# stdstu12/YUME

Measured on NVIDIA H100. Metric: latent_frames_per_sec, higher is better.
Workload: dtype bf16

## Files before the change

include/yume_b200.h:

```cpp
#ifndef YUME_B200_H_
#define YUME_B200_H_

#ifdef __cplusplus
extern "C" {
#endif

#define YB_OK 0
#define YB_ERR_ARG (-1)
#define YB_ERR_SHAPE (-2)
#define YB_ERR_ALIGNMENT (-3)
#define YB_ERR_NO_DRIVER (-4)
#define YB_ERR_TENSORMAP (-5)
#define YB_ERR_LAUNCH (-6)

int yb_abi_version(void);

#define YB_EPI_BF16 0
#define YB_EPI_GELU_BF16 1
#define YB_EPI_F32 2
#define YB_EPI_GATE_RES 3
#define YB_EPI_RES_BF16 5
#define YB_EPI_GELU_ERF_BF16 4

typedef struct yb_gemm_args {
// ... 15 lines not shown
  long long a_split_stride;
  const void* res;
  long long res_ld;
  int split_k;
  void* ws;
  long long ws_bytes;
} yb_gemm_args;
int yb_gemm_bf16(const yb_gemm_args* args, void* stream);
long long yb_gemm_workspace_bytes(int M, int N, int K, int epilogue, int cta_pair, int split_k);
int yb_gemm_splitk_plan(int tiles, int num_kb, int clusters, int split_k, int* out3);
int yb_gemm_plan(int M, int N, int sms, int* out4);

typedef struct yb_conv3d_args {
  unsigned int struct_bytes;
  int cta_pair;
  const void* xpad;
  const void* w;
  const void* bias;
  void* out;
  const void* res;
  long long ldo, res_ld;
  int T, H, W, Cp, Cout;
  int epilogue;
  int kt, kh, kw;
  int oob_zero_pad;
  int out_t_mul, out_t_add;
  int fuse_w;
  int stride_t, stride_hw;
} yb_conv3d_args;
int yb_conv3d_causal(const yb_conv3d_args* args, void* stream);
int yb_conv3d_plan(int T, int H, int W, int Cout, int kw, int fuse_w, int* out4);

int yb_ln_modulate(const void* x, long long ldx, void* out, long long ldo, int out_f32, const void* scale,
                   const void* shift, long long mod_ld, const void* tok_idx, const void* weight, const void* lnbias,
                   int L, int C, float eps, void* stream);

int yb_rmsnorm_rope(void* qk, long long ld, const void* weight, const void* rope, int rope_len, int L, int C, int D,
                    float eps, void* stream);
int yb_rmsnorm_rope_pieces(void* qk, long long ld, int piece_cols, long long piece_stride, const void* weight,
                           const void* rope, int rope_len, int L, int C, int D, float eps, void* stream);

int yb_qk_norm_rope(void* q, void* k, long long ld, int piece_cols, long long piece_stride, const void* wq, const void* wk,
                    const void* rope, int rope_len, int L, int C, int D, float eps, void* stream);

int yb_attention(const void* q, long long ldq, const void* k, long long ldk, const void* v, long long ldv, void* out,
                 long long ldo, int Lq, int Lk, int heads, float scale, int flags, void* stream);
int yb_attention_ex(const void* q, long long ldq, const void* k, long long ldk, const void* v, long long ldv, void* out,
                    long long ldo, int Lq, int Lk, int heads, float scale, int flags, void* ws, long long ws_bytes,
                    void* trace, void* stream);
#define YB_ATT_P_SMEM 1
#define YB_ATT_EMU_SHIFT 2
#define YB_ATT_ACCUMULATE 2
#define YB_ATT_SPLIT_SHIFT 4
int yb_attention_plan(int Lq, int Lk, int heads, int sms, int flags, int* out4);
long long yb_attention_workspace_bytes(int Lq, int Lk, int heads, int sms, int flags);
int yb_debug_force_split(int ns);
int yb_sp_scatter_qkv(const void* qkv, long long ld, const void* wq, const void* wk, const void* rope, int rope_len,
                      int L, int C, int D, float eps, void* const* peers, int world, int rank, int Lp, void* stream);
int yb_gemm_sp_qkv(const void* A, long long lda, const void* W, const void* bias, int Lp_rows, int C, int K, void* const* peers,
                   int world, int rank, int Lp, void* sums, void* stream);
int yb_sp_bcast_sums(void* local_sums, void* const* peer_tables, int world, int rank, int Lp, void* stream);
int yb_sp_post_norm_rope(void* buf, const void* sums, const void* wq, const void* wk, const void* rope, int rope_len, int L,
                         int Wh, int C, int D, float eps, void* stream);
int yb_attention_sp(const void* q, long long ldq, const void* k, long long ldk, const void* v, long long ldv,
                    void* const* out_peers, long long ldo, int Lq, int Lk, int heads, float scale, int world, int rank,
                    int Lp, int flags, void* ws, long long ws_bytes, void* stream);

int yb_patchify(const void* x, long long sc, long long sf, long long sh, long long sw, void* out, long long ldo,
                int Cin, int F, int H, int W, int ph, int pw, void* stream);

int yb_unpatchify(const void* y, long long ldy, void* out, int Cout, int F, int Hp, int Wp, int ph, int pw,
                  void* stream);

int yb_bcast_add(const void* a, const void* b, void* out, int R1, int R2, int n, void* stream);

int yb_sinusoidal(const void* t, void* out, int n, int dim, void* stream);

int yb_linear_f32_small(const void* in, const void* W, const void* bias, void* out, int M, int N, int K, int silu_in,
                        void* stream);

int yb_linear_f32(const void* in, long long ldi, const void* W, const void* bias, void* out, long long ldo, int M,
                  int N, int K, void* stream);

int yb_gn_stats(const void* x, long long ld, void* stats, long long N, int C, int G, void* stream);
int yb_vae_pad_act(const void* x, long long ldx, int Ts, int Hs, int Ws, int C, void* out, int Cp, int pad, int ft, int fh,
                   int fw, const void* stats, const void* gamma, const void* beta, int G, float eps, int silu,
                   void* stream);
int yb_masked_softmax(const void* S, long long ldS, void* P, long long ldP, int L, int hw, void* stream);
int yb_nchw_to_nhwc_bf16(const void* x, void* out, long long N, int Cn, int ldo, void* stream);
int yb_nhwc_to_nchw_f32(const void* x, long long ldx, void* out, long long N, int Cn, void* stream);
int yb_nhwc_to_nchw_f32_clamp(const void* x, long long ldx, void* out, long long N, int Cn, float lo, float hi, void* stream);
int yb_blend(const void* a, void* b, long long outer, int ea, int eb, int ext, long long inner, void* stream);

int yb_vae_assemble_tiles(const void* const* tile_ptrs, const int* th, const int* tw, const int* tlen, const int* tf0, int nt,
                          int ni, int nj, int C, int F, int H, int W, int row_limit, int blend_extent, int t_limit,
                          int t_blend_extent, void* out, void* stream);

int yb_vae_rms_act(const void* x, long long ldx, void* out, const void* gamma, int T, int Hs, int Ws, int C, int Cp, int up,
                   int silu, void* stream);
int yb_vae_dupup_add(void* main_, const void* x, int Ts, int Hs, int Ws, int in_c, int out_c, int ft, int fs, void* stream);
int yb_vae_unpatchify2_clamp(const void* y, long long ldy, void* out, int T, int H, int W, void* stream);
int yb_vae_avgdown_add(void* main_, const void* x, int T, int H, int W, int in_c, int out_c, int ft, int fs, void* stream);
int yb_vae_patchify2_bf16(const void* video, void* out, long long ldo, int T, int H, int W, void* stream);

int yb_umma_probe(const void* A, const void* B, void* D, int mode, void* stream);

// ... 5 lines not shown
```

yume_b200/_lib.py:

```python
from __future__ import annotations

import ctypes as C
from pathlib import Path

_LIB_PATH = Path(__file__).resolve().parent / "csrc" / "libyume_b200.so"

YB_EPI_BF16, YB_EPI_GELU_BF16, YB_EPI_F32, YB_EPI_GATE_RES, YB_EPI_GELU_ERF_BF16, YB_EPI_RES_BF16 = 0, 1, 2, 3, 4, 5
YB_ATT_P_SMEM, YB_ATT_ACCUMULATE = 1, 2
ABI_VERSION = 4
YB_ATT_EMU_SHIFT, YB_ATT_SPLIT_SHIFT = 2, 4

_ERRORS = {
    -1: "YB_ERR_ARG (null pointer / bad enum / non-positive size)",
    -2: "YB_ERR_SHAPE (shape not supported by the kernel)",
    -3: "YB_ERR_ALIGNMENT (pointer or stride not 16-byte aligned)",
    -4: "YB_ERR_NO_DRIVER (cuTensorMapEncodeTiled unavailable: no CUDA driver)",
    -5: "YB_ERR_TENSORMAP (driver rejected a TMA descriptor)",
    -6: "YB_ERR_LAUNCH (kernel launch failed)",
}


class YumeB200Error(RuntimeError):
    pass


class GemmArgs(C.Structure):

    _fields_ = [
        ("struct_bytes", C.c_uint), ("cta_pair", C.c_int),
        ("A", C.c_void_p), ("B", C.c_void_p), ("bias", C.c_void_p), ("out", C.c_void_p),
        ("gate", C.c_void_p), ("tok_idx", C.c_void_p),
        ("lda", C.c_longlong), ("ldb", C.c_longlong), ("ldo", C.c_longlong), ("gate_ld", C.c_longlong),
        ("M", C.c_int), ("N", C.c_int), ("K", C.c_int), ("epilogue", C.c_int), ("block_n", C.c_int),
        ("n_split", C.c_int), ("split_stride", C.c_longlong), ("a_split", C.c_int), ("a_split_stride", C.c_longlong),
        ("res", C.c_void_p), ("res_ld", C.c_longlong),
        ("split_k", C.c_int), ("ws", C.c_void_p), ("ws_bytes", C.c_longlong),
    ]


class Conv3dArgs(C.Structure):

    _fields_ = [
        ("struct_bytes", C.c_uint), ("cta_pair", C.c_int),
        ("xpad", C.c_void_p), ("w", C.c_void_p), ("bias", C.c_void_p), ("out", C.c_void_p), ("res", C.c_void_p),
        ("ldo", C.c_longlong), ("res_ld", C.c_longlong),
        ("T", C.c_int), ("H", C.c_int), ("W", C.c_int), ("Cp", C.c_int), ("Cout", C.c_int), ("epilogue", C.c_int),
        ("kt", C.c_int), ("kh", C.c_int), ("kw", C.c_int), ("oob_zero_pad", C.c_int), ("out_t_mul", C.c_int),
        ("out_t_add", C.c_int), ("fuse_w", C.c_int), ("stride_t", C.c_int), ("stride_hw", C.c_int),
    ]


_vp, _ll, _i, _f = C.c_void_p, C.c_longlong, C.c_int, C.c_float
SIGNATURES = {
    "yb_abi_version": (_i, []),
    "yb_gemm_bf16": (_i, [C.POINTER(GemmArgs), _vp]),
    "yb_conv3d_causal": (_i, [C.POINTER(Conv3dArgs), _vp]),
    "yb_gn_stats": (_i, [_vp, _ll, _vp, _ll, _i, _i, _vp]),
    "yb_vae_pad_act": (_i, [_vp, _ll, _i, _i, _i, _i, _vp, _i, _i, _i, _i, _i, _vp, _vp, _vp, _i, _f, _i, _vp]),
    "yb_masked_softmax": (_i, [_vp, _ll, _vp, _ll, _i, _i, _vp]),
    "yb_nchw_to_nhwc_bf16": (_i, [_vp, _vp, _ll, _i, _i, _vp]),
    "yb_nhwc_to_nchw_f32": (_i, [_vp, _ll, _vp, _ll, _i, _vp]),
# ... 71 lines not shown
```

yume_b200/csrc/attention.cu:

```cuda
#include "yb_host.h"
#include "yb_ptx.cuh"

namespace yb {

constexpr int ATT_THREADS = 384;
constexpr int ATT_TILE_BYTES = 128 * 128 * 2;

struct AttParams {
  __nv_bfloat16* out;
  long long ldo;
  int Lq, Lk;
  int nkv;
  int accumulate;
  __nv_bfloat16* out_peers[8];
  int sp_world, sp_rank, sp_Lp;
  float scale_log2;
  int nq, full_units, ns;
  float* ws_o;
  float* ws_ml;
};

template <bool P_SMEM>
struct AttCfg {
  static constexpr int NS = P_SMEM ? 4 : 5;
  static constexpr int Q_OFF = 0;
  static constexpr int P_OFF = ATT_TILE_BYTES;
  static constexpr int KV_OFF = P_SMEM ? 2 * ATT_TILE_BYTES : ATT_TILE_BYTES;
  static constexpr int BAR_OFF = KV_OFF + NS * ATT_TILE_BYTES;
  static constexpr int SMEM_BYTES = BAR_OFF + 256 + 1024;
  static_assert(SMEM_BYTES <= 227 * 1024, "shared memory budget");
};

template <bool P_SMEM>
__global__ void __launch_bounds__(ATT_THREADS, 1)
attention_kernel(const __grid_constant__ CUtensorMap tmQ, const __grid_constant__ CUtensorMap tmK,
                 const __grid_constant__ CUtensorMap tmV, const AttParams p) {
  using Cfg = AttCfg<P_SMEM>;
  constexpr int NS = Cfg::NS;
  extern __shared__ uint8_t smem_raw[];
  uint8_t* smem = reinterpret_cast<uint8_t*>((reinterpret_cast<uintptr_t>(smem_raw) + 1023) & ~uintptr_t(1023));
  uint64_t* q_full = reinterpret_cast<uint64_t*>(smem + Cfg::BAR_OFF);
  uint64_t* q_empty = q_full + 1;
  uint64_t* kv_full = q_empty + 1;
  uint64_t* kv_empty = kv_full + NS;

  const int warp = threadIdx.x >> 5;
  const int lane = threadIdx.x & 31;
  int unit = blockIdx.x, kv_begin = 0, nkv = p.nkv;
  if (static_cast<int>(blockIdx.x) >= p.full_units) {
    const int r = blockIdx.x - p.full_units;
    unit = p.full_units + r / p.ns;
    const int per = (((p.nkv + p.ns - 1) / p.ns) + 1) & ~1;
    kv_begin = (r % p.ns) * per;
    nkv = min(per, p.nkv - kv_begin);
  }
  const int head = unit / p.nq;
  const int q0 = (unit - head * p.nq) * 256;
  const int nx = q0 + 128 < p.Lq ? 2 : 1;

  if (threadIdx.x == 0) {
    tma_prefetch_desc(&tmQ);
    tma_prefetch_desc(&tmK);
    tma_prefetch_desc(&tmV);
    mbar_init(q_full, 1);
    mbar_init(q_empty, 8);
    for (int i = 0; i < NS; ++i) {
      mbar_init(&kv_full[i], 1);
      mbar_init(&kv_empty[i], 8);
    }
    fence_barrier_init();
  }
  __syncthreads();

  if (warp < 4) {
    setmaxnreg_dec<40>();
    if (warp == 0 && lane == 0) {
      int it = 0;
      for (int X = 0; X < nx; ++X) {
        if (X == 1) mbar_wait(q_empty, 0);
        mbar_arrive_expect_tx(q_full, ATT_TILE_BYTES);
        for (int s = 0; s < 2; ++s)
          tma_load_2d(smem + Cfg::Q_OFF + s * 16384, &tmQ, q_full, head * 128 + s * 64, q0 + X * 128);
        for (int jj = 0; jj < 2 * nkv; ++jj, ++it) {
          const int slot = it % NS;
          mbar_wait(&kv_empty[slot], ((it / NS) & 1) ^ 1);
          mbar_arrive_expect_tx(&kv_full[slot], ATT_TILE_BYTES);
          const CUtensorMap* tm = (jj & 1) ? &tmV : &tmK;
          uint8_t* dst = smem + Cfg::KV_OFF + slot * ATT_TILE_BYTES;
          const int j = kv_begin + (jj >> 1);
          tma_load_2d(dst, tm, &kv_full[slot], head * 128, j * 128);
          tma_load_2d(dst + 16384, tm, &kv_full[slot], head * 128 + 64, j * 128);
        }
      }
    }
  } else {
    setmaxnreg_inc<232>();
    const int wg = (warp >> 2) - 1;
    const int q4 = lane >> 2, c2 = 2 * (lane & 3);
    const int row_a = wg * 64 + (warp & 3) * 16 + q4;
    const float sc = p.scale_log2;
    const uint32_t sQ = smem_u32(smem + Cfg::Q_OFF) + wg * 64 * 128;
    const uint32_t sP = smem_u32(smem + Cfg::P_OFF) + wg * 16384;
    int it = 0;
    for (int X = 0; X < nx; ++X) {
      mbar_wait(q_full, X);
      float o[64];
#pragma unroll
      for (int i = 0; i < 64; ++i) o[i] = 0.f;
      float m0 = -INFINITY, m1 = -INFINITY, l0 = 0.f, l1 = 0.f;
      for (int j = 0; j < nkv; ++j, it += 2) {
        const int slot_k = it % NS, slot_v = (it + 1) % NS;
        mbar_wait(&kv_full[slot_k], (it / NS) & 1);
        const uint32_t sK = smem_u32(smem + Cfg::KV_OFF + slot_k * ATT_TILE_BYTES);
        float s[64];
#pragma unroll
        for (int i = 0; i < 64; ++i) s[i] = 0.f;
        wgmma_fence();
#pragma unroll
        for (int kk = 0; kk < 8; ++kk) {
          const uint32_t off = (kk >> 2) * 16384 + (kk & 3) * 32;
          wgmma_ss_acc64<0>(s, make_smem_desc_sw128(sQ + off, 16, 1024), make_smem_desc_sw128(sK + off, 16, 1024), kk != 0);
        }
        wgmma_commit();
        wgmma_wait<0>();
        fence_regs(s);
        __syncwarp();
        if (lane == 0) {
          mbar_arrive(&kv_empty[slot_k]);
          if (j == nkv - 1) mbar_arrive(q_empty);
        }
        const int kv_rem = p.Lk - (kv_begin + j) * 128;
        if (kv_rem < 128) {
#pragma unroll
          for (int i = 0; i < 64; ++i)
            if (8 * (i >> 2) + c2 + (i & 1) >= kv_rem) s[i] = -INFINITY;
        }
        float mx0 = -INFINITY, mx1 = -INFINITY;
#pragma unroll
        for (int g = 0; g < 16; ++g) {
          mx0 = fmaxf(mx0, fmaxf(s[4 * g], s[4 * g + 1]));
          mx1 = fmaxf(mx1, fmaxf(s[4 * g + 2], s[4 * g + 3]));
        }
        mx0 = fmaxf(mx0, __shfl_xor_sync(0xffffffffu, mx0, 1));
        mx0 = fmaxf(mx0, __shfl_xor_sync(0xffffffffu, mx0, 2));
        mx1 = fmaxf(mx1, __shfl_xor_sync(0xffffffffu, mx1, 1));
        mx1 = fmaxf(mx1, __shfl_xor_sync(0xffffffffu, mx1, 2));
        const float mn0 = fmaxf(m0, mx0 * sc), mn1 = fmaxf(m1, mx1 * sc);
        const float al0 = fast_exp2(m0 - mn0), al1 = fast_exp2(m1 - mn1);
        m0 = mn0;
        m1 = mn1;
        l0 *= al0;
        l1 *= al1;
#pragma unroll
        for (int g = 0; g < 16; ++g) {
          o[4 * g] *= al0;
          o[4 * g + 1] *= al0;
          o[4 * g + 2] *= al1;
          o[4 * g + 3] *= al1;
        }
        uint32_t pa[8][4];
#pragma unroll
        for (int kk = 0; kk < 8; ++kk) {
          float e[8];
#pragma unroll
          for (int i = 0; i < 8; ++i) e[i] = fast_exp2(s[8 * kk + i] * sc - ((i & 2) ? m1 : m0));
          l0 += (e[0] + e[1]) + (e[4] + e[5]);
          l1 += (e[2] + e[3]) + (e[6] + e[7]);
          pa[kk][0] = pack_bf16x2(e[0], e[1]);
          pa[kk][1] = pack_bf16x2(e[2], e[3]);
          pa[kk][2] = pack_bf16x2(e[4], e[5]);
          pa[kk][3] = pack_bf16x2(e[6], e[7]);
        }
        if (P_SMEM) {
          const int ra = row_a - wg * 64, rb = ra + 8;
#pragma unroll
          for (int kk = 0; kk < 8; ++kk) {
            uint8_t* slab = smem + Cfg::P_OFF + wg * 16384 + (kk >> 2) * 8192;
            const int k0 = (kk & 3) * 16 + c2, k1 = k0 + 8;
            *reinterpret_cast<uint32_t*>(slab + ra * 128 + (((k0 >> 3) ^ (ra & 7)) << 4) + (k0 & 7) * 2) = pa[kk][0];
            *reinterpret_cast<uint32_t*>(slab + rb * 128 + (((k0 >> 3) ^ (rb & 7)) << 4) + (k0 & 7) * 2) = pa[kk][1];
            *reinterpret_cast<uint32_t*>(slab + ra * 128 + (((k1 >> 3) ^ (ra & 7)) << 4) + (k1 & 7) * 2) = pa[kk][2];
            *reinterpret_cast<uint32_t*>(slab + rb * 128 + (((k1 >> 3) ^ (rb & 7)) << 4) + (k1 & 7) * 2) = pa[kk][3];
          }
          fence_proxy_async_smem();
          named_bar_sync(1 + wg, 128);
        }
        mbar_wait(&kv_full[slot_v], ((it + 1) / NS) & 1);
        const uint32_t sV = smem_u32(smem + Cfg::KV_OFF + slot_v * ATT_TILE_BYTES);
        wgmma_fence();
#pragma unroll
        for (int kk = 0; kk < 8; ++kk) {
          const uint64_t vdesc = make_smem_desc_sw128(sV + kk * 2048, 16384, 1024);
          if (P_SMEM)
            wgmma_ss_acc64<1>(o, make_smem_desc_sw128(sP + (kk >> 2) * 8192 + (kk & 3) * 32, 16, 1024), vdesc, 1u);
          else
            wgmma_rs_n128_tb(o, pa[kk], vdesc, 1u);
        }
        wgmma_commit();
        wgmma_wait<0>();
        fence_regs(o);
        __syncwarp();
        if (lane == 0) mbar_arrive(&kv_empty[slot_v]);
      }
      l0 += __shfl_xor_sync(0xffffffffu, l0, 1);
      l0 += __shfl_xor_sync(0xffffffffu, l0, 2);
      l1 += __shfl_xor_sync(0xffffffffu, l1, 1);
      l1 += __shfl_xor_sync(0xffffffffu, l1, 2);

#pragma unroll
      for (int h = 0; h < 2; ++h) {
        const int row_t = X * 128 + row_a + 8 * h;
        const float m = h ? m1 : m0, l = h ? l1 : l0;
        if (static_cast<int>(blockIdx.x) >= p.full_units) {
          const long long prow = static_cast<long long>(blockIdx.x - p.full_units) * 256 + row_t;
          float* wo = p.ws_o + prow * 128;
#pragma unroll
          for (int g = 0; g < 16; ++g) *reinterpret_cast<float2*>(wo + 8 * g + c2) = make_float2(o[4 * g + 2 * h], o[4 * g + 2 * h + 1]);
          if ((lane & 3) == 0) *reinterpret_cast<float2*>(p.ws_ml + prow * 2) = make_float2(m, l);
          continue;
        }
        const int q_row = q0 + row_t;
        if (q_row >= p.Lq) continue;
        __nv_bfloat16* orow = p.out + static_cast<long long>(q_row) * p.ldo + head * 128;
        if (p.sp_world > 1) {
          const int owner = q_row / p.sp_Lp;
          const int t = q_row - owner * p.sp_Lp;
          if (owner < p.sp_world)
            orow = p.out_peers[owner] + (static_cast<long long>(p.sp_rank) * p.sp_Lp + t) * p.ldo + head * 128;
        }
        const float inv = 1.0f / l;
#pragma unroll
        for (int g = 0; g < 16; ++g) {
          uint32_t* dst = reinterpret_cast<uint32_t*>(orow + 8 * g + c2);
          float v0 = o[4 * g + 2 * h] * inv, v1 = o[4 * g + 2 * h + 1] * inv;
          if (p.accumulate) {
            const float2 prev = __bfloat1622float2(*reinterpret_cast<const __nv_bfloat162*>(dst));
            v0 += prev.x;
            v1 += prev.y;
          }
          *dst = pack_bf16x2(v0, v1);
        }
      }
    }
  }
}

__global__ void __launch_bounds__(256) attention_combine_kernel(const AttParams p, int tail_units) {
  const int gw = blockIdx.x * 8 + (threadIdx.x >> 5);
  const int lane = threadIdx.x & 31;
  if (gw >= tail_units * 256) return;
  const int tu = gw >> 8, r = gw & 255;
  const int unit = p.full_units + tu;
  const int head = unit / p.nq;
  const int q_row = (unit - head * p.nq) * 256 + r;
  if (q_row >= p.Lq) return;
  float M = -INFINITY;
  for (int sgm = 0; sgm < p.ns; ++sgm) M = fmaxf(M, p.ws_ml[((static_cast<long long>(tu) * p.ns + sgm) * 256 + r) * 2]);
  float4 acc = make_float4(0.f, 0.f, 0.f, 0.f);
  float lsum = 0.f;
  for (int sgm = 0; sgm < p.ns; ++sgm) {
    const long long prow = (static_cast<long long>(tu) * p.ns + sgm) * 256 + r;
    const float2 ml = *reinterpret_cast<const float2*>(p.ws_ml + prow * 2);
    const float w = exp2f(ml.x - M);
    const float4 o = *reinterpret_cast<const float4*>(p.ws_o + prow * 128 + lane * 4);
    acc.x += o.x * w; acc.y += o.y * w; acc.z += o.z * w; acc.w += o.w * w;
    lsum += ml.y * w;
  }
  const float inv = 1.0f / lsum;
  __nv_bfloat16* orow = p.out + static_cast<long long>(q_row) * p.ldo + head * 128;
  if (p.sp_world > 1) {
    const int owner = q_row / p.sp_Lp;
    const int t = q_row - owner * p.sp_Lp;
    if (owner < p.sp_world)
      orow = p.out_peers[owner] + (static_cast<long long>(p.sp_rank) * p.sp_Lp + t) * p.ldo + head * 128;
  }
  *reinterpret_cast<uint2*>(orow + lane * 4) = make_uint2(pack_bf16x2(acc.x * inv, acc.y * inv), pack_bf16x2(acc.z * inv, acc.w * inv));
}

static void attention_plan(int units, int nkv, int sms, bool allowed, int force_ns, int* full_units, int* tail, int* ns) {
  *full_units = units;
  *tail = 0;
  *ns = 1;
  if (!allowed || force_ns == 1) return;
  if (force_ns >= 2 && nkv >= 2 * force_ns) {
    *tail = units;
    *ns = force_ns;
  } else if (force_ns == 0 && units > sms && units % sms != 0 && 2 * (units % sms) <= sms && nkv >= 16) {
    *tail = units % sms;
    *ns = sms / *tail < 4 ? sms / *tail : 4;
  }
  while (*ns > 1 && (*ns - 1) * ((((nkv + *ns - 1) / *ns) + 1) & ~1) >= nkv) --*ns;
  if (*ns == 1) *tail = 0;
  *full_units = units - *tail;
}

static size_t split_workspace_bytes(size_t ctas) { return ctas * 256 * 130 * sizeof(float); }

static int g_debug_force_split = 0;

template <bool P_SMEM>
static int launch_attention(const CUtensorMap& tmQ, const CUtensorMap& tmK, const CUtensorMap& tmV,
                            AttParams p, int heads, cudaStream_t stream, int force_ns, void* ws, long long ws_bytes) {
  using Cfg = AttCfg<P_SMEM>;
  auto kern = attention_kernel<P_SMEM>;
  static bool attr_set[kMaxDevices] = {false};
  if (int rc = ensure_dynamic_smem(kern, Cfg::SMEM_BYTES, attr_set, "attention")) return rc;
  if (force_ns == 0 && g_debug_force_split >= 1 && g_debug_force_split <= 4) force_ns = g_debug_force_split;
  p.nq = (p.Lq + 255) / 256;
  const int units = p.nq * heads;
  int tail = 0;
  p.ws_o = p.ws_ml = nullptr;
  const bool allowed = !p.accumulate && ws != nullptr;
  attention_plan(units, p.nkv, sm_count(), allowed, force_ns, &p.full_units, &tail, &p.ns);
  if (tail > 0) {
    const size_t ctas = static_cast<size_t>(tail) * p.ns;
    if (ws_bytes < 0 || static_cast<size_t>(ws_bytes) < split_workspace_bytes(ctas) || (reinterpret_cast<uintptr_t>(ws) & 0xF)) {
      p.full_units = units;
      tail = 0;
      p.ns = 1;
    } else {
      p.ws_o = static_cast<float*>(ws);
      p.ws_ml = p.ws_o + ctas * 256 * 128;
    }
  }
  kern<<<p.full_units + tail * p.ns, ATT_THREADS, Cfg::SMEM_BYTES, stream>>>(tmQ, tmK, tmV, p);
  int rc = check_launch("attention");
  if (rc || tail == 0) return rc;
  attention_combine_kernel<<<tail * 32, 256, 0, stream>>>(p, tail);
  return check_launch("attention_combine");
}

static int dispatch_attention(const void* q, long long ldq, const void* k, long long ldk, const void* v, long long ldv,
                              AttParams p, int heads, cudaStream_t stream, int flags, void* ws, long long ws_bytes) {
  const int force_ns = (flags >> YB_ATT_SPLIT_SHIFT) & 7;
  if (force_ns > 4) return YB_ERR_ARG;
  if ((flags >> YB_ATT_EMU_SHIFT) & 3) return YB_ERR_ARG;
  CUtensorMap tmQ, tmK, tmV;
  const uint64_t cols = static_cast<uint64_t>(heads) * 128;
  int rc = make_tmap_bf16_2d(&tmQ, q, p.Lq, cols, ldq, 128, 64);
  if (rc) return rc;
  rc = make_tmap_bf16_2d(&tmK, k, p.Lk, cols, ldk, 128, 64);
  if (rc) return rc;
  rc = make_tmap_bf16_2d(&tmV, v, p.Lk, cols, ldv, 128, 64);
  if (rc) return rc;
  if (flags & YB_ATT_P_SMEM) return launch_attention<true>(tmQ, tmK, tmV, p, heads, stream, force_ns, ws, ws_bytes);
  return launch_attention<false>(tmQ, tmK, tmV, p, heads, stream, force_ns, ws, ws_bytes);
}

}

extern "C" int yb_debug_force_split(int ns) {
  if (ns < 0 || ns > 4) return YB_ERR_ARG;
  yb::g_debug_force_split = ns;
  return YB_OK;
}

extern "C" int yb_attention_plan(int Lq, int Lk, int heads, int sms, int flags, int* out4) {
  if (Lq <= 0 || Lk <= 0 || heads <= 0 || sms <= 0 || !out4) return YB_ERR_ARG;
  int force_ns = (flags >> YB_ATT_SPLIT_SHIFT) & 7;
  if (force_ns > 4) return YB_ERR_ARG;
  if (force_ns == 0 && yb::g_debug_force_split >= 1) force_ns = yb::g_debug_force_split;
  const int nkv = (Lk + 127) / 128;
  int full_units, tail, ns;
  yb::attention_plan(((Lq + 255) / 256) * heads, nkv, sms, !(flags & YB_ATT_ACCUMULATE), force_ns, &full_units, &tail, &ns);
  out4[0] = full_units;
  out4[1] = tail;
  out4[2] = ns;
  out4[3] = ns > 1 ? ((((nkv + ns - 1) / ns) + 1) & ~1) : nkv;
  return YB_OK;
}

extern "C" long long yb_attention_workspace_bytes(int Lq, int Lk, int heads, int sms, int flags) {
  int plan[4];
  if (yb_attention_plan(Lq, Lk, heads, sms, flags, plan)) return -1;
  return static_cast<long long>(yb::split_workspace_bytes(static_cast<size_t>(plan[1]) * plan[2]));
}

extern "C" int yb_attention_ex(const void* q, long long ldq, const void* k, long long ldk, const void* v,
                               long long ldv, void* out, long long ldo, int Lq, int Lk, int heads, float scale,
                               int flags, void* ws, long long ws_bytes, void* trace, void* stream_) {
  using namespace yb;
  if (!q || !k || !v || !out) return YB_ERR_ARG;
  if (Lq <= 0 || Lk <= 0 || heads <= 0) return YB_ERR_ARG;
  if ((ldo % 8) != 0 || (reinterpret_cast<uintptr_t>(out) & 0xF)) return YB_ERR_ALIGNMENT;
  AttParams p;
  p.out = static_cast<__nv_bfloat16*>(out);
  p.ldo = ldo;
  p.Lq = Lq;
  p.Lk = Lk;
  p.nkv = (Lk + 127) / 128;
  p.accumulate = (flags & YB_ATT_ACCUMULATE) ? 1 : 0;
  (void)trace;
  p.sp_world = 1;
  p.sp_rank = 0;
  p.sp_Lp = 0;
  p.scale_log2 = scale * 1.4426950408889634f;
  return dispatch_attention(q, ldq, k, ldk, v, ldv, p, heads, reinterpret_cast<cudaStream_t>(stream_), flags, ws, ws_bytes);
}

// ... 28 lines not shown
```

yume_b200/ops.py:

```python
from __future__ import annotations

import ctypes as C
import math
from typing import Optional

import torch

from . import _lib
from ._lib import (YB_ATT_ACCUMULATE, YB_ATT_P_SMEM, YB_EPI_BF16, YB_EPI_F32, YB_EPI_GATE_RES, YB_EPI_GELU_BF16,
                   YB_EPI_GELU_ERF_BF16, YB_EPI_RES_BF16, Conv3dArgs, GemmArgs, YumeB200Error, check)

__all__ = [
    "gemm", "ln_modulate", "rmsnorm_rope", "qk_norm_rope", "flop_count", "attention", "patchify", "unpatchify", "sinusoidal",
    "resize_bicubic_normalize",
    "linear_f32_small", "linear_f32", "umma_probe", "launch_count", "reset_launch_count",
    "YB_EPI_BF16", "YB_EPI_GELU_BF16", "YB_EPI_F32", "YB_EPI_GATE_RES", "YB_EPI_GELU_ERF_BF16", "bcast_add",
    "YB_ATT_P_SMEM", "YB_ATT_ACCUMULATE",
]

_launches = 0
_flops = 0.0


def flop_count() -> float:
    return _flops


def launch_count() -> int:
    return _launches


def reset_launch_count() -> None:
    global _launches, _flops
    _launches = 0
    _flops = 0.0


def _stream() -> int:
    return torch.cuda.current_stream().cuda_stream


def _ptr(t: Optional[torch.Tensor]) -> Optional[int]:
    return None if t is None else t.data_ptr()


def _need(t: torch.Tensor, dtype, name: str) -> None:
    if not t.is_cuda:
        raise YumeB200Error(f"{name} must be a CUDA tensor (yume_b200 has no CPU path)")
    if t.dtype != dtype:
        raise YumeB200Error(f"{name} must be {dtype}, got {t.dtype}")
    if t.stride(-1) != 1:
        raise YumeB200Error(f"{name} must be contiguous in its last dimension")


def gemm(a: torch.Tensor, w: torch.Tensor, bias: Optional[torch.Tensor], out: torch.Tensor, epilogue: int,
         gate: Optional[torch.Tensor] = None, tok_idx: Optional[torch.Tensor] = None, block_n: int = 0,
         n_split: int = 0, split_stride: int = 0, a_split: int = 0, a_split_stride: int = 0,
         shape: Optional[tuple] = None, res: Optional[torch.Tensor] = None, cta_pair: int = 0, split_k: Optional[int] = None) -> torch.Tensor:
    global _launches, _flops
    _need(a, torch.bfloat16, "a")
    _need(w, torch.bfloat16, "w")
    N, K2 = w.shape
    if shape is not None:
        M, K = shape
    else:
        M, K = a.shape
    if K2 != K:
        raise YumeB200Error(f"gemm K mismatch: {K} vs {K2}")
    want = torch.bfloat16 if epilogue in (YB_EPI_BF16, YB_EPI_GELU_BF16, YB_EPI_GELU_ERF_BF16, YB_EPI_RES_BF16) else torch.float32
    if res is not None:
# ... 67 lines not shown
    check(_lib.load().yb_rmsnorm_rope_pieces(qk.data_ptr(), qk.stride(0), piece_cols, piece_stride, weight.data_ptr(),
                                             _ptr(rope), rope_len or 0, L, Cdim, head_dim, eps, _stream()),
          "yb_rmsnorm_rope")
    _launches += 1
    return qk


def qk_norm_rope(q: torch.Tensor, k: torch.Tensor, wq: torch.Tensor, wk: torch.Tensor, rope: Optional[torch.Tensor],
                 head_dim: int, eps: float = 1e-6, rope_len: Optional[int] = None, pieces: Optional[tuple] = None) -> None:
    global _launches
    _need(q, torch.bfloat16, "q")
    _need(k, torch.bfloat16, "k")
    _need(wq, torch.float32, "wq")
    _need(wk, torch.float32, "wk")
    if q.stride(0) != k.stride(0):
        raise YumeB200Error("q and k must share their row stride")
    if pieces is not None:
        L, Cdim, piece_cols, piece_stride = pieces
    else:
        if q.shape != k.shape:
            raise YumeB200Error("q and k must have the same shape")
        L, Cdim = q.shape
        piece_cols, piece_stride = Cdim, 0
    if rope is not None:
        _need(rope, torch.float32, "rope")
        if not rope.is_contiguous() or rope.shape[-1] != 2 or rope.shape[-2] != head_dim // 2:
            raise YumeB200Error("rope must be contiguous f32 [L, D/2, 2]")
        if rope_len is None:
            rope_len = rope.shape[0]
    check(_lib.load().yb_qk_norm_rope(q.data_ptr(), k.data_ptr(), q.stride(0), piece_cols, piece_stride, wq.data_ptr(),
                                      wk.data_ptr(), _ptr(rope), rope_len or 0, L, Cdim, head_dim, eps, _stream()),
          "yb_qk_norm_rope")
    _launches += 1


_sm_counts = {}


def _sms(device: torch.device) -> int:
    idx = device.index if device.index is not None else torch.cuda.current_device()
    n = _sm_counts.get(idx)
    if n is None:
        n = _sm_counts[idx] = torch.cuda.get_device_properties(idx).multi_processor_count
    return n


def _attention_ws(Lq: int, Lk: int, heads: int, flags: int, device: torch.device):
    nbytes = _lib.load().yb_attention_workspace_bytes(Lq, Lk, heads, _sms(device), flags)
    if nbytes <= 0:
        return None, 0
    return torch.empty(nbytes, dtype=torch.uint8, device=device), nbytes


def attention(q: torch.Tensor, k: torch.Tensor, v: torch.Tensor, out: torch.Tensor, heads: int,
              scale: Optional[float] = None, variant: int = 0, accumulate: bool = False,
              split: int = 0) -> torch.Tensor:
    global _launches, _flops
    for n, t in (("q", q), ("k", k), ("v", v), ("out", out)):
        _need(t, torch.bfloat16, n)
    Lq, Lk = q.shape[0], k.shape[0]
    if q.shape[1] != heads * 128 or k.shape[1] != heads * 128 or v.shape[1] != heads * 128:
        raise YumeB200Error("attention supports head_dim 128 only")
    if scale is None:
        scale = 1.0 / math.sqrt(128.0)
    flags = (YB_ATT_P_SMEM if variant == 1 else 0) | (YB_ATT_ACCUMULATE if accumulate else 0) | ((split & 7) << 4)
    if variant not in (0, 1):
        raise YumeB200Error("attention variant must be 0 or 1")
    ws, ws_bytes = _attention_ws(Lq, Lk, heads, flags, q.device)
    check(_lib.load().yb_attention_ex(q.data_ptr(), q.stride(0), k.data_ptr(), k.stride(0), v.data_ptr(), v.stride(0),
                                      out.data_ptr(), out.stride(0), Lq, Lk, heads, scale, flags, _ptr(ws), ws_bytes, None,
                                      _stream()), "yb_attention")
    _launches += 1
    _flops += 4.0 * Lq * Lk * heads * 128
    return out


def patchify(x: torch.Tensor, out: torch.Tensor, ph: int, pw: int) -> torch.Tensor:
    global _launches
    if not x.is_cuda or x.dtype != torch.float32:
        raise YumeB200Error("patchify input must be a CUDA float32 tensor")
    _need(out, torch.bfloat16, "out")
    Cin, F, H, W = x.shape
    sc, sf, sh, sw = x.stride()
    check(_lib.load().yb_patchify(x.data_ptr(), sc, sf, sh, sw, out.data_ptr(), out.stride(0), Cin, F, H, W, ph, pw,
                                  _stream()), "yb_patchify")
    _launches += 1
    return out


def resize_bicubic_normalize(x: torch.Tensor, out: torch.Tensor, mean: torch.Tensor, std: torch.Tensor) -> torch.Tensor:
    global _launches
    if not x.is_cuda or x.dtype != torch.float32 or x.dim() != 3:
        raise YumeB200Error("resize_bicubic_normalize input must be a CUDA float32 [C, H, W] tensor")
    _need(out, torch.float32, "out")
    Cn, H, W = x.shape
    S = out.shape[-1]
    if not out.is_contiguous() or tuple(out.shape) != (Cn, S, S):
        raise YumeB200Error(f"resize_bicubic_normalize out must be a contiguous [{Cn}, S, S], got {tuple(out.shape)}")
    for name, t in (("mean", mean), ("std", std)):
        _need(t, torch.float32, name)
        if t.numel() != Cn or not t.is_contiguous():
            raise YumeB200Error(f"resize_bicubic_normalize {name} must be a contiguous f32 [{Cn}]")
    sc, sh, sw = x.stride()
    check(_lib.load().yb_resize_bicubic_normalize(x.data_ptr(), sc, sh, sw, Cn, H, W, out.data_ptr(), S, mean.data_ptr(),
                                                  std.data_ptr(), _stream()), "yb_resize_bicubic_normalize")
    _launches += 1
    return out


def unpatchify(y: torch.Tensor, out: torch.Tensor, F: int, Hp: int, Wp: int, ph: int, pw: int) -> torch.Tensor:
    global _launches
    _need(y, torch.float32, "y")
    _need(out, torch.float32, "out")
    Cout = out.shape[0]
    check(_lib.load().yb_unpatchify(y.data_ptr(), y.stride(0), out.data_ptr(), Cout, F, Hp, Wp, ph, pw, _stream()),
          "yb_unpatchify")
    _launches += 1
    return out


# ... 207 lines not shown


def _ptr_array(ptrs):
    arr = (C.c_void_p * len(ptrs))(*[int(p) for p in ptrs])
    return arr


def sp_scatter_qkv(qkv: torch.Tensor, wq: torch.Tensor, wk: torch.Tensor, rope: Optional[torch.Tensor], rope_len: int,
                   head_dim: int, eps: float, peer_ptrs, rank: int, Lp: int) -> None:
    global _launches
    _need(qkv, torch.bfloat16, "qkv")
    L, C3 = qkv.shape
    check(_lib.load().yb_sp_scatter_qkv(qkv.data_ptr(), qkv.stride(0), wq.data_ptr(), wk.data_ptr(), _ptr(rope), rope_len,
                                        L, C3 // 3, head_dim, eps, _ptr_array(peer_ptrs), len(peer_ptrs), rank, Lp,
                                        _stream()), "yb_sp_scatter_qkv")
    _launches += 1


def gemm_sp_qkv(h: torch.Tensor, w_qkv: torch.Tensor, b_qkv: torch.Tensor, peer_ptrs, rank: int, Lp: int,
                sums: torch.Tensor) -> None:
    global _launches, _flops
    _need(h, torch.bfloat16, "h")
    _need(w_qkv, torch.bfloat16, "w_qkv")
    _need(b_qkv, torch.float32, "b_qkv")
    _need(sums, torch.float32, "sums")
    if not w_qkv.is_contiguous():
        raise YumeB200Error("gemm_sp_qkv weight must be contiguous")
    M, K = h.shape
    C3 = w_qkv.shape[0]
    check(_lib.load().yb_gemm_sp_qkv(h.data_ptr(), h.stride(0), w_qkv.data_ptr(), b_qkv.data_ptr(), M, C3 // 3, K,
                                     _ptr_array(peer_ptrs), len(peer_ptrs), rank, Lp, sums.data_ptr(), _stream()),
          "yb_gemm_sp_qkv")
    _launches += 1
    _flops += 2.0 * M * C3 * K


def sp_bcast_sums(local: torch.Tensor, peer_table_ptrs, rank: int, Lp: int) -> None:
    global _launches
    check(_lib.load().yb_sp_bcast_sums(local.data_ptr(), _ptr_array(peer_table_ptrs), len(peer_table_ptrs), rank, Lp, _stream()),
          "yb_sp_bcast_sums")
    _launches += 1


def sp_post_norm_rope(buf: torch.Tensor, sums: torch.Tensor, wq: torch.Tensor, wk: torch.Tensor, rope: Optional[torch.Tensor],
                      rope_len: int, L: int, Wh: int, Cdim: int, head_dim: int, eps: float) -> None:
    global _launches
    _need(buf, torch.bfloat16, "buf")
    check(_lib.load().yb_sp_post_norm_rope(buf.data_ptr(), sums.data_ptr(), wq.data_ptr(), wk.data_ptr(), _ptr(rope), rope_len, L,
                                           Wh, Cdim, head_dim, eps, _stream()), "yb_sp_post_norm_rope")
    _launches += 1


def attention_sp(q: torch.Tensor, k: torch.Tensor, v: torch.Tensor, out_peer_ptrs, ldo: int, heads: int, rank: int,
                 Lp: int, scale: Optional[float] = None) -> None:
    global _launches, _flops
    for n, t in (("q", q), ("k", k), ("v", v)):
        _need(t, torch.bfloat16, n)
    if scale is None:
        scale = 1.0 / math.sqrt(128.0)
    flags = 0
    ws, ws_bytes = _attention_ws(q.shape[0], k.shape[0], heads, flags, q.device)
    check(_lib.load().yb_attention_sp(q.data_ptr(), q.stride(0), k.data_ptr(), k.stride(0), v.data_ptr(), v.stride(0),
                                      _ptr_array(out_peer_ptrs), ldo, q.shape[0], k.shape[0], heads, scale,
                                      len(out_peer_ptrs), rank, Lp, flags, _ptr(ws), ws_bytes, _stream()), "yb_attention_sp")
    _launches += 1
    _flops += 4.0 * q.shape[0] * k.shape[0] * heads * 128


def vae_rms_act(x: torch.Tensor, dims, out: torch.Tensor, gamma: Optional[torch.Tensor], up: int = 1, silu: bool = True) -> torch.Tensor:
    global _launches
    _need(x, torch.bfloat16, "x")
    _need(out, torch.bfloat16, "out")
    T, Hs, Ws = dims
    if not out.is_contiguous():
        raise YumeB200Error("vae_rms_act output must be contiguous")
    check(_lib.load().yb_vae_rms_act(x.data_ptr(), x.stride(0), out.data_ptr(), _ptr(gamma), T, Hs, Ws, x.shape[1],
                                     out.shape[-1], up, 1 if silu else 0, _stream()), "yb_vae_rms_act")
    _launches += 1
    return out


def vae_dupup_add(main: torch.Tensor, x: torch.Tensor, dims, in_c: int, out_c: int, ft: int, fs: int) -> torch.Tensor:
    global _launches
    _need(main, torch.bfloat16, "main")
    _need(x, torch.bfloat16, "x")
    if not (main.is_contiguous() and x.is_contiguous()):
        raise YumeB200Error("vae_dupup_add needs dense tensors")
    check(_lib.load().yb_vae_dupup_add(main.data_ptr(), x.data_ptr(), dims[0], dims[1], dims[2], in_c, out_c, ft, fs,
                                       _stream()), "yb_vae_dupup_add")
    _launches += 1
    return main


def vae_avgdown_add(main: torch.Tensor, x: torch.Tensor, dims, in_c: int, out_c: int, ft: int, fs: int) -> torch.Tensor:
    global _launches
    _need(main, torch.bfloat16, "main")
    _need(x, torch.bfloat16, "x")
    if not (main.is_contiguous() and x.is_contiguous()) or x.shape[-1] != in_c or main.shape[-1] != out_c:
        raise YumeB200Error("vae_avgdown_add needs dense [.., in_c] / [.., out_c] tensors")
    check(_lib.load().yb_vae_avgdown_add(main.data_ptr(), x.data_ptr(), dims[0], dims[1], dims[2], in_c, out_c, ft, fs,
                                         _stream()), "yb_vae_avgdown_add")
    _launches += 1
    return main


def vae_patchify2_bf16(video: torch.Tensor, out: torch.Tensor) -> torch.Tensor:
    global _launches
    _need(video, torch.float32, "video")
    _need(out, torch.bfloat16, "out")
    if video.dim() != 4 or video.shape[0] != 3 or not video.is_contiguous() or not out.is_contiguous():
        raise YumeB200Error("vae_patchify2_bf16: video must be a contiguous [3, T, H, W]")
    _, T, H, W = video.shape
    check(_lib.load().yb_vae_patchify2_bf16(video.data_ptr(), out.data_ptr(), out.shape[-1], T, H, W, _stream()),
# ... 14 lines not shown
```

Before: 39.05.

## Pipeline attention QK^T of next tile with PV of previous tile

Adds a software-pipelined attention schedule in which the QK^T wgmma for tile j is issued together with the PV wgmma for tile j-1, so softmax overlaps with tensor-core work. P is passed through shared memory in this path. The old serial schedule stays available behind a new SERIAL flag, and the default variant now runs the pipelined P-in-smem kernel instead of the register-P kernel. This adds shared-memory stores of P and extra synchronization, and may raise register pressure.

```diff
diff --git a/include/yume_b200.h b/include/yume_b200.h
--- a/include/yume_b200.h
+++ b/include/yume_b200.h
@@ -91,6 +91,7 @@
 #define YB_ATT_EMU_SHIFT 2
 #define YB_ATT_ACCUMULATE 2
 #define YB_ATT_SPLIT_SHIFT 4
+#define YB_ATT_SERIAL 128
 int yb_attention_plan(int Lq, int Lk, int heads, int sms, int flags, int* out4);
 long long yb_attention_workspace_bytes(int Lq, int Lk, int heads, int sms, int flags);
 int yb_debug_force_split(int ns);
diff --git a/yume_b200/_lib.py b/yume_b200/_lib.py
--- a/yume_b200/_lib.py
+++ b/yume_b200/_lib.py
@@ -6,7 +6,7 @@
 _LIB_PATH = Path(__file__).resolve().parent / "csrc" / "libyume_b200.so"
 
 YB_EPI_BF16, YB_EPI_GELU_BF16, YB_EPI_F32, YB_EPI_GATE_RES, YB_EPI_GELU_ERF_BF16, YB_EPI_RES_BF16 = 0, 1, 2, 3, 4, 5
-YB_ATT_P_SMEM, YB_ATT_ACCUMULATE = 1, 2
+YB_ATT_P_SMEM, YB_ATT_ACCUMULATE, YB_ATT_SERIAL = 1, 2, 128
 ABI_VERSION = 4
 YB_ATT_EMU_SHIFT, YB_ATT_SPLIT_SHIFT = 2, 4
 
diff --git a/yume_b200/csrc/attention.cu b/yume_b200/csrc/attention.cu
--- a/yume_b200/csrc/attention.cu
+++ b/yume_b200/csrc/attention.cu
@@ -31,10 +31,100 @@
   static_assert(SMEM_BYTES <= 227 * 1024, "shared memory budget");
 };
 
+__device__ __forceinline__ void att_issue_qk(float (&s)[64], uint32_t sQ, uint32_t sK) {
+#pragma unroll
+  for (int i = 0; i < 64; ++i) s[i] = 0.f;
+  wgmma_fence();
+#pragma unroll
+  for (int kk = 0; kk < 8; ++kk) {
+    const uint32_t off = (kk >> 2) * 16384 + (kk & 3) * 32;
+    wgmma_ss_acc64<0>(s, make_smem_desc_sw128(sQ + off, 16, 1024), make_smem_desc_sw128(sK + off, 16, 1024), kk != 0);
+  }
+  wgmma_commit();
+}
+
+__device__ __forceinline__ void att_softmax(float (&s)[64], int kv_rem, int c2, float sc, float& m0, float& m1, float& l0,
+                                            float& l1, float& al0, float& al1, uint32_t (&pa)[8][4]) {
+  if (kv_rem < 128) {
+#pragma unroll
+    for (int i = 0; i < 64; ++i)
+      if (8 * (i >> 2) + c2 + (i & 1) >= kv_rem) s[i] = -INFINITY;
+  }
+  float mx0 = -INFINITY, mx1 = -INFINITY;
+#pragma unroll
+  for (int g = 0; g < 16; ++g) {
+    mx0 = fmaxf(mx0, fmaxf(s[4 * g], s[4 * g + 1]));
+    mx1 = fmaxf(mx1, fmaxf(s[4 * g + 2], s[4 * g + 3]));
+  }
+  mx0 = fmaxf(mx0, __shfl_xor_sync(0xffffffffu, mx0, 1));
+  mx0 = fmaxf(mx0, __shfl_xor_sync(0xffffffffu, mx0, 2));
+  mx1 = fmaxf(mx1, __shfl_xor_sync(0xffffffffu, mx1, 1));
+  mx1 = fmaxf(mx1, __shfl_xor_sync(0xffffffffu, mx1, 2));
+  const float mn0 = fmaxf(m0, mx0 * sc), mn1 = fmaxf(m1, mx1 * sc);
+  al0 = fast_exp2(m0 - mn0);
+  al1 = fast_exp2(m1 - mn1);
+  m0 = mn0;
+  m1 = mn1;
+  l0 *= al0;
+  l1 *= al1;
+#pragma unroll
+  for (int kk = 0; kk < 8; ++kk) {
+    float e[8];
+#pragma unroll
+    for (int i = 0; i < 8; ++i) e[i] = fast_exp2(s[8 * kk + i] * sc - ((i & 2) ? m1 : m0));
+    l0 += (e[0] + e[1]) + (e[4] + e[5]);
+    l1 += (e[2] + e[3]) + (e[6] + e[7]);
+    pa[kk][0] = pack_bf16x2(e[0], e[1]);
+    pa[kk][1] = pack_bf16x2(e[2], e[3]);
+    pa[kk][2] = pack_bf16x2(e[4], e[5]);
+    pa[kk][3] = pack_bf16x2(e[6], e[7]);
+  }
+}
+
+__device__ __forceinline__ void att_rescale(float (&o)[64], float al0, float al1) {
+#pragma unroll
+  for (int g = 0; g < 16; ++g) {
+    o[4 * g] *= al0;
+    o[4 * g + 1] *= al0;
+    o[4 * g + 2] *= al1;
+    o[4 * g + 3] *= al1;
+  }
+}
+
 template <bool P_SMEM>
+__device__ __forceinline__ void att_issue_pv(float (&o)[64], const uint32_t (&pa)[8][4], uint32_t sP, uint32_t sV) {
+  wgmma_fence();
+#pragma unroll
+  for (int kk = 0; kk < 8; ++kk) {
+    const uint64_t vdesc = make_smem_desc_sw128(sV + kk * 2048, 16384, 1024);
+    if (P_SMEM)
+      wgmma_ss_acc64<1>(o, make_smem_desc_sw128(sP + (kk >> 2) * 8192 + (kk & 3) * 32, 16, 1024), vdesc, 1u);
+    else
+      wgmma_rs_n128_tb(o, pa[kk], vdesc, 1u);
+  }
+  wgmma_commit();
+}
+
+__device__ __forceinline__ void att_store_p(uint32_t sP, int ra, int c2, int wg, const uint32_t (&pa)[8][4]) {
+  const uint32_t row = sP + ra * 128 + c2 * 2, x = (ra & 7) << 4;
+#pragma unroll
+  for (int kk = 0; kk < 8; ++kk) {
+    const uint32_t a0 = row + (kk >> 2) * 8192 + (((kk & 3) * 32) ^ x);
+    const uint32_t a1 = row + (kk >> 2) * 8192 + (((kk & 3) * 32 + 16) ^ x);
+    asm volatile("st.shared.b32 [%0], %1;" ::"r"(a0), "r"(pa[kk][0]) : "memory");
+    asm volatile("st.shared.b32 [%0], %1;" ::"r"(a0 + 1024), "r"(pa[kk][1]) : "memory");
+    asm volatile("st.shared.b32 [%0], %1;" ::"r"(a1), "r"(pa[kk][2]) : "memory");
+    asm volatile("st.shared.b32 [%0], %1;" ::"r"(a1 + 1024), "r"(pa[kk][3]) : "memory");
+  }
+  fence_proxy_async_smem();
+  named_bar_sync(1 + wg, 128);
+}
+
+template <bool P_SMEM, bool SERIAL>
 __global__ void __launch_bounds__(ATT_THREADS, 1)
 attention_kernel(const __grid_constant__ CUtensorMap tmQ, const __grid_constant__ CUtensorMap tmK,
                  const __grid_constant__ CUtensorMap tmV, const AttParams p) {
+  static_assert(SERIAL || P_SMEM, "the pipelined schedule passes P through shared memory");
   using Cfg = AttCfg<P_SMEM>;
   constexpr int NS = Cfg::NS;
   extern __shared__ uint8_t smem_raw[];
@@ -101,6 +191,7 @@
     const float sc = p.scale_log2;
     const uint32_t sQ = smem_u32(smem + Cfg::Q_OFF) + wg * 64 * 128;
     const uint32_t sP = smem_u32(smem + Cfg::P_OFF) + wg * 16384;
+    auto kv_smem = [&](int slot) { return smem_u32(smem + Cfg::KV_OFF + slot * ATT_TILE_BYTES); };
     int it = 0;
     for (int X = 0; X < nx; ++X) {
       mbar_wait(q_full, X);
@@ -108,95 +199,77 @@
 #pragma unroll
       for (int i = 0; i < 64; ++i) o[i] = 0.f;
       float m0 = -INFINITY, m1 = -INFINITY, l0 = 0.f, l1 = 0.f;
-      for (int j = 0; j < nkv; ++j, it += 2) {
-        const int slot_k = it % NS, slot_v = (it + 1) % NS;
-        mbar_wait(&kv_full[slot_k], (it / NS) & 1);
-        const uint32_t sK = smem_u32(smem + Cfg::KV_OFF + slot_k * ATT_TILE_BYTES);
-        float s[64];
-#pragma unroll
-        for (int i = 0; i < 64; ++i) s[i] = 0.f;
-        wgmma_fence();
-#pragma unroll
-        for (int kk = 0; kk < 8; ++kk) {
-          const uint32_t off = (kk >> 2) * 16384 + (kk & 3) * 32;
-          wgmma_ss_acc64<0>(s, make_smem_desc_sw128(sQ + off, 16, 1024), make_smem_desc_sw128(sK + off, 16, 1024), kk != 0);
-        }
-        wgmma_commit();
-        wgmma_wait<0>();
-        fence_regs(s);
-        __syncwarp();
-        if (lane == 0) {
-          mbar_arrive(&kv_empty[slot_k]);
-          if (j == nkv - 1) mbar_arrive(q_empty);
-        }
-        const int kv_rem = p.Lk - (kv_begin + j) * 128;
-        if (kv_rem < 128) {
-#pragma unroll
-          for (int i = 0; i < 64; ++i)
-            if (8 * (i >> 2) + c2 + (i & 1) >= kv_rem) s[i] = -INFINITY;
-        }
-        float mx0 = -INFINITY, mx1 = -INFINITY;
-#pragma unroll
-        for (int g = 0; g < 16; ++g) {
-          mx0 = fmaxf(mx0, fmaxf(s[4 * g], s[4 * g + 1]));
-          mx1 = fmaxf(mx1, fmaxf(s[4 * g + 2], s[4 * g + 3]));
-        }
-        mx0 = fmaxf(mx0, __shfl_xor_sync(0xffffffffu, mx0, 1));
-        mx0 = fmaxf(mx0, __shfl_xor_sync(0xffffffffu, mx0, 2));
-        mx1 = fmaxf(mx1, __shfl_xor_sync(0xffffffffu, mx1, 1));
-        mx1 = fmaxf(mx1, __shfl_xor_sync(0xffffffffu, mx1, 2));
-        const float mn0 = fmaxf(m0, mx0 * sc), mn1 = fmaxf(m1, mx1 * sc);
-        const float al0 = fast_exp2(m0 - mn0), al1 = fast_exp2(m1 - mn1);
-        m0 = mn0;
-        m1 = mn1;
-        l0 *= al0;
-        l1 *= al1;
-#pragma unroll
-        for (int g = 0; g < 16; ++g) {
-          o[4 * g] *= al0;
-          o[4 * g + 1] *= al0;
-          o[4 * g + 2] *= al1;
-          o[4 * g + 3] *= al1;
-        }
+      if constexpr (SERIAL) {
+        for (int j = 0; j < nkv; ++j, it += 2) {
+          const int slot_k = it % NS, slot_v = (it + 1) % NS;
+          mbar_wait(&kv_full[slot_k], (it / NS) & 1);
+          float s[64];
+          att_issue_qk(s, sQ, kv_smem(slot_k));
+          wgmma_wait<0>();
+          fence_regs(s);
+          __syncwarp();
+          if (lane == 0) {
+            mbar_arrive(&kv_empty[slot_k]);
+            if (j == nkv - 1) mbar_arrive(q_empty);
+          }
+          float al0, al1;
+          uint32_t pa[8][4];
+          att_softmax(s, p.Lk - (kv_begin + j) * 128, c2, sc, m0, m1, l0, l1, al0, al1, pa);
+          att_rescale(o, al0, al1);
+          if (P_SMEM) att_store_p(sP, row_a - wg * 64, c2, wg, pa);
+          mbar_wait(&kv_full[slot_v], ((it + 1) / NS) & 1);
+          att_issue_pv<P_SMEM>(o, pa, sP, kv_smem(slot_v));
+          wgmma_wait<0>();
+          fence_regs(o);
+          __syncwarp();
+          if (lane == 0) mbar_arrive(&kv_empty[slot_v]);
+        }
+      } else {
         uint32_t pa[8][4];
-#pragma unroll
-        for (int kk = 0; kk < 8; ++kk) {
-          float e[8];
-#pragma unroll
-          for (int i = 0; i < 8; ++i) e[i] = fast_exp2(s[8 * kk + i] * sc - ((i & 2) ? m1 : m0));
-          l0 += (e[0] + e[1]) + (e[4] + e[5]);
-          l1 += (e[2] + e[3]) + (e[6] + e[7]);
-          pa[kk][0] = pack_bf16x2(e[0], e[1]);
-          pa[kk][1] = pack_bf16x2(e[2], e[3]);
-          pa[kk][2] = pack_bf16x2(e[4], e[5]);
-          pa[kk][3] = pack_bf16x2(e[6], e[7]);
-        }
-        if (P_SMEM) {
-          const int ra = row_a - wg * 64, rb = ra + 8;
-#pragma unroll
-          for (int kk = 0; kk < 8; ++kk) {
-            uint8_t* slab = smem + Cfg::P_OFF + wg * 16384 + (kk >> 2) * 8192;
-            const int k0 = (kk & 3) * 16 + c2, k1 = k0 + 8;
-            *reinterpret_cast<uint32_t*>(slab + ra * 128 + (((k0 >> 3) ^ (ra & 7)) << 4) + (k0 & 7) * 2) = pa[kk][0];
-            *reinterpret_cast<uint32_t*>(slab + rb * 128 + (((k0 >> 3) ^ (rb & 7)) << 4) + (k0 & 7) * 2) = pa[kk][1];
-            *reinterpret_cast<uint32_t*>(slab + ra * 128 + (((k1 >> 3) ^ (ra & 7)) << 4) + (k1 & 7) * 2) = pa[kk][2];
-            *reinterpret_cast<uint32_t*>(slab + rb * 128 + (((k1 >> 3) ^ (rb & 7)) << 4) + (k1 & 7) * 2) = pa[kk][3];
+        {
+          const int slot_k = it % NS;
+          mbar_wait(&kv_full[slot_k], (it / NS) & 1);
+          float s[64];
+          att_issue_qk(s, sQ, kv_smem(slot_k));
+          wgmma_wait<0>();
+          fence_regs(s);
+          __syncwarp();
+          if (lane == 0) {
+            mbar_arrive(&kv_empty[slot_k]);
+            if (nkv == 1) mbar_arrive(q_empty);
           }
-          fence_proxy_async_smem();
-          named_bar_sync(1 + wg, 128);
-        }
-        mbar_wait(&kv_full[slot_v], ((it + 1) / NS) & 1);
-        const uint32_t sV = smem_u32(smem + Cfg::KV_OFF + slot_v * ATT_TILE_BYTES);
-        wgmma_fence();
-#pragma unroll
-        for (int kk = 0; kk < 8; ++kk) {
-          const uint64_t vdesc = make_smem_desc_sw128(sV + kk * 2048, 16384, 1024);
-          if (P_SMEM)
-            wgmma_ss_acc64<1>(o, make_smem_desc_sw128(sP + (kk >> 2) * 8192 + (kk & 3) * 32, 16, 1024), vdesc, 1u);
-          else
-            wgmma_rs_n128_tb(o, pa[kk], vdesc, 1u);
-        }
-        wgmma_commit();
+          float al0, al1;
+          att_softmax(s, p.Lk - kv_begin * 128, c2, sc, m0, m1, l0, l1, al0, al1, pa);
+          att_rescale(o, al0, al1);
+          att_store_p(sP, row_a - wg * 64, c2, wg, pa);
+          it += 2;
+        }
+        for (int j = 1; j < nkv; ++j, it += 2) {
+          const int slot_k = it % NS, slot_v = (it + NS - 1) % NS;
+          mbar_wait(&kv_full[slot_k], (it / NS) & 1);
+          float s[64];
+          att_issue_qk(s, sQ, kv_smem(slot_k));
+          mbar_wait(&kv_full[slot_v], ((it - 1) / NS) & 1);
+          att_issue_pv<true>(o, pa, sP, kv_smem(slot_v));
+          wgmma_wait<1>();
+          fence_regs(s);
+          __syncwarp();
+          if (lane == 0) {
+            mbar_arrive(&kv_empty[slot_k]);
+            if (j == nkv - 1) mbar_arrive(q_empty);
+          }
+          float al0, al1;
+          att_softmax(s, p.Lk - (kv_begin + j) * 128, c2, sc, m0, m1, l0, l1, al0, al1, pa);
+          wgmma_wait<0>();
+          fence_regs(o);
+          __syncwarp();
+          if (lane == 0) mbar_arrive(&kv_empty[slot_v]);
+          att_rescale(o, al0, al1);
+          att_store_p(sP, row_a - wg * 64, c2, wg, pa);
+        }
+        const int slot_v = (it - 1) % NS;
+        mbar_wait(&kv_full[slot_v], ((it - 1) / NS) & 1);
+        att_issue_pv<true>(o, pa, sP, kv_smem(slot_v));
         wgmma_wait<0>();
         fence_regs(o);
         __syncwarp();
@@ -298,11 +371,11 @@
 
 static int g_debug_force_split = 0;
 
-template <bool P_SMEM>
+template <bool P_SMEM, bool SERIAL>
 static int launch_attention(const CUtensorMap& tmQ, const CUtensorMap& tmK, const CUtensorMap& tmV,
                             AttParams p, int heads, cudaStream_t stream, int force_ns, void* ws, long long ws_bytes) {
   using Cfg = AttCfg<P_SMEM>;
-  auto kern = attention_kernel<P_SMEM>;
+  auto kern = attention_kernel<P_SMEM, SERIAL>;
   static bool attr_set[kMaxDevices] = {false};
   if (int rc = ensure_dynamic_smem(kern, Cfg::SMEM_BYTES, attr_set, "attention")) return rc;
   if (force_ns == 0 && g_debug_force_split >= 1 && g_debug_force_split <= 4) force_ns = g_debug_force_split;
@@ -343,8 +416,9 @@
   if (rc) return rc;
   rc = make_tmap_bf16_2d(&tmV, v, p.Lk, cols, ldv, 128, 64);
   if (rc) return rc;
-  if (flags & YB_ATT_P_SMEM) return launch_attention<true>(tmQ, tmK, tmV, p, heads, stream, force_ns, ws, ws_bytes);
-  return launch_attention<false>(tmQ, tmK, tmV, p, heads, stream, force_ns, ws, ws_bytes);
+  if (flags & YB_ATT_P_SMEM) return launch_attention<true, true>(tmQ, tmK, tmV, p, heads, stream, force_ns, ws, ws_bytes);
+  if (flags & YB_ATT_SERIAL) return launch_attention<false, true>(tmQ, tmK, tmV, p, heads, stream, force_ns, ws, ws_bytes);
+  return launch_attention<true, false>(tmQ, tmK, tmV, p, heads, stream, force_ns, ws, ws_bytes);
 }
 
 }
diff --git a/yume_b200/ops.py b/yume_b200/ops.py
--- a/yume_b200/ops.py
+++ b/yume_b200/ops.py
@@ -7,7 +7,7 @@
 import torch
 
 from . import _lib
-from ._lib import (YB_ATT_ACCUMULATE, YB_ATT_P_SMEM, YB_EPI_BF16, YB_EPI_F32, YB_EPI_GATE_RES, YB_EPI_GELU_BF16,
+from ._lib import (YB_ATT_ACCUMULATE, YB_ATT_P_SMEM, YB_ATT_SERIAL, YB_EPI_BF16, YB_EPI_F32, YB_EPI_GATE_RES, YB_EPI_GELU_BF16,
                    YB_EPI_GELU_ERF_BF16, YB_EPI_RES_BF16, Conv3dArgs, GemmArgs, YumeB200Error, check)
 
 __all__ = [
@@ -15,7 +15,7 @@
     "resize_bicubic_normalize",
     "linear_f32_small", "linear_f32", "umma_probe", "launch_count", "reset_launch_count",
     "YB_EPI_BF16", "YB_EPI_GELU_BF16", "YB_EPI_F32", "YB_EPI_GATE_RES", "YB_EPI_GELU_ERF_BF16", "bcast_add",
-    "YB_ATT_P_SMEM", "YB_ATT_ACCUMULATE",
+    "YB_ATT_P_SMEM", "YB_ATT_ACCUMULATE", "YB_ATT_SERIAL",
 ]
 
 _launches = 0
@@ -189,6 +189,9 @@
     return torch.empty(nbytes, dtype=torch.uint8, device=device), nbytes
 
 
+_ATT_VARIANT_FLAGS = {0: 0, 1: YB_ATT_P_SMEM, 2: YB_ATT_SERIAL}
+
+
 def attention(q: torch.Tensor, k: torch.Tensor, v: torch.Tensor, out: torch.Tensor, heads: int,
               scale: Optional[float] = None, variant: int = 0, accumulate: bool = False,
               split: int = 0) -> torch.Tensor:
@@ -200,9 +203,9 @@
         raise YumeB200Error("attention supports head_dim 128 only")
     if scale is None:
         scale = 1.0 / math.sqrt(128.0)
-    flags = (YB_ATT_P_SMEM if variant == 1 else 0) | (YB_ATT_ACCUMULATE if accumulate else 0) | ((split & 7) << 4)
-    if variant not in (0, 1):
-        raise YumeB200Error("attention variant must be 0 or 1")
+    if variant not in (0, 1, 2):
+        raise YumeB200Error("attention variant must be 0, 1 or 2")
+    flags = _ATT_VARIANT_FLAGS[variant] | (YB_ATT_ACCUMULATE if accumulate else 0) | ((split & 7) << 4)
     ws, ws_bytes = _attention_ws(Lq, Lk, heads, flags, q.device)
     check(_lib.load().yb_attention_ex(q.data_ptr(), q.stride(0), k.data_ptr(), k.stride(0), v.data_ptr(), v.stride(0),
                                       out.data_ptr(), out.stride(0), Lq, Lk, heads, scale, flags, _ptr(ws), ws_bytes, None,
@@ -516,13 +519,15 @@
 
 
 def attention_sp(q: torch.Tensor, k: torch.Tensor, v: torch.Tensor, out_peer_ptrs, ldo: int, heads: int, rank: int,
-                 Lp: int, scale: Optional[float] = None) -> None:
+                 Lp: int, scale: Optional[float] = None, variant: int = 0) -> None:
     global _launches, _flops
+    if variant not in (0, 2):
+        raise YumeB200Error("attention_sp variant must be 0 or 2")
     for n, t in (("q", q), ("k", k), ("v", v)):
         _need(t, torch.bfloat16, n)
     if scale is None:
         scale = 1.0 / math.sqrt(128.0)
-    flags = 0
+    flags = _ATT_VARIANT_FLAGS[variant]
     ws, ws_bytes = _attention_ws(q.shape[0], k.shape[0], heads, flags, q.device)
     check(_lib.load().yb_attention_sp(q.data_ptr(), q.stride(0), k.data_ptr(), k.stride(0), v.data_ptr(), v.stride(0),
                                       _ptr_array(out_peer_ptrs), ldo, q.shape[0], k.shape[0], heads, scale,
```

New measurement: 39.17 (median of 6 runs). Within noise of the previous version (+0.3%).
